# element36-io/hyperfridge-r0

Hardware: AMD Instinct MI355X
Metric: segments/sec (po2=20) proving camt53 guest, 1/2/4/8 MI355X (higher is better)
Workload: dtype u32

## Files before the change

hyperfridge-r0_amd/csrc/circuit.hip:

```cpp
#include <hip/hiprtc.h>

#include <memory>

#include "circuit.hpp"

namespace r0h {

static const char* compile_in_process(const std::string& src, std::vector<char>& code) {
  hiprtcProgram prog;
  hiprtcResult r = hiprtcCreateProgram(&prog, src.c_str(), "eval_check.hip", 0, nullptr, nullptr);
  R0H_REQUIRE(r == HIPRTC_SUCCESS, "hiprtcCreateProgram: %s", hiprtcGetErrorString(r));
  const char* opts[] = {"--offload-arch=gfx950", "-O3"};
  r = hiprtcCompileProgram(prog, 2, opts);
  if (r != HIPRTC_SUCCESS) {
    size_t n = 0;
    hiprtcGetProgramLogSize(prog, &n);
    std::string log(n, 0);
    if (n) hiprtcGetProgramLog(prog, &log[0]);
    hiprtcDestroyProgram(&prog);
    return make_error("hiprtcCompileProgram: %s\n%.2000s", hiprtcGetErrorString(r), log.c_str());
  }
  size_t n = 0;
  hiprtcGetCodeSize(prog, &n);
  code.resize(n);
// ... 80 lines not shown
  kernels_out->swap(kernels);
  return nullptr;
}

const char* r0h_circuit_load(r0h_ctx* ctx, const uint32_t* blob, size_t n_words, const char* code_object_path, r0h_circuit** out) {
  R0H_GUARD_BEGIN
  R0H_REQUIRE(ctx && blob && out, "r0h_circuit_load: NULL argument");
  std::unique_ptr<r0h_circuit, CircuitUnload> c(new r0h_circuit());
  c->ctx = ctx;
  R0H_TRY(parse_blob(c.get(), blob, n_words));
  make_plan(c.get());
  R0H_TRY(load_module("r0h_circuit_load", c.get(), code_object_path, emit_source, "eval_check", c->plan.terms.empty() ? 0 : 1, true, &c->module, &c->kernels));
  ctx_retain(ctx);
  *out = c.release();
  return nullptr;
  R0H_GUARD_END
}

const char* r0h_circuit_free(r0h_circuit* c) {
  if (!c) return nullptr;
  r0h_ctx* ctx = c->ctx;
  (void)hipSetDevice(ctx->device);
  (void)hipStreamSynchronize(ctx->stream);
  CircuitUnload()(c);
  ctx_release(ctx);
  return nullptr;
}

uint32_t r0h_circuit_group_size(const r0h_circuit* c, uint32_t group) { return c && group < 3 ? c->group_size[group] : 0; }
uint32_t r0h_circuit_n_global(const r0h_circuit* c) { return c ? c->n_global : 0; }
uint32_t r0h_circuit_n_mix(const r0h_circuit* c) { return c ? c->n_mix : 0; }
uint32_t r0h_circuit_n_taps(const r0h_circuit* c) { return c ? (uint32_t)c->taps.size() : 0; }
uint32_t r0h_circuit_n_terms(const r0h_circuit* c) { return c ? (uint32_t)c->plan.terms.size() : 0; }

static const char* check_module_load(const r0h_circuit* c, const char* caller, const char* code_object_path) {
  if (c->check_module) return nullptr;
  return load_module(caller, c, code_object_path, emit_check_source, "check_witness", c->plan.cut.size() - 1, false, &c->check_module, &c->check_kernels);
}

const char* r0h_circuit_load_check(r0h_circuit* c, const char* code_object_path) {
  R0H_GUARD_BEGIN
  R0H_REQUIRE(c, "r0h_circuit_load_check: NULL argument");
  std::lock_guard<std::mutex> lk(c->check_mu);
  R0H_REQUIRE(!c->check_module, "r0h_circuit_load_check: the circuit's checker is loaded already");
  return check_module_load(c, "r0h_circuit_load_check", code_object_path);
  R0H_GUARD_END
// ... 23 lines not shown
  const size_t table_at = kinds.size();
  for (uint32_t v : c->periodic) kinds.push_back(enc(v));
  R0H_TRY(ensure_scratch(ctx, kinds.size() * 4));
  R0H_TRY(stage_h2d(ctx, ctx->scratch, kinds.data(), kinds.size() * 4));
  const uint32_t* dk = (const uint32_t*)ctx->scratch;
  hipLaunchKernelGGL(witgen_fixed_kernel, dim3(n / threads, cols), dim3(threads), 0, ctx->stream, u32(buf), dk, po2, seed_mixed, dk + table_at, c->period);
  return launch_ok("r0h_witgen");
}
const char* witgen_code(r0h_ctx* ctx, const r0h_circuit* c, uint32_t po2, r0h_buf* code) {
  R0H_REQUIRE(ctx && c && code, "r0h_witgen: NULL argument");
  R0H_REQUIRE(c->has_column_program, "r0h_witgen: this circuit carries no synthetic column program (WITGEN/ACCUM sections); supply the witness");
  R0H_REQUIRE(po2 >= 4 && po2 <= R0H_MAX_PO2, "r0h_witgen: po2 %u outside [4, %u]", po2, R0H_MAX_PO2);
  const uint32_t nc = (uint32_t)c->code_cols.size();
  R0H_REQUIRE(((size_t)nc << po2) * 4 <= code->bytes, "r0h_witgen: buffers too small for 2^%u rows", po2);
  std::vector<uint32_t> kinds(2 * (size_t)nc);
  for (uint32_t k = 0; k < nc; k++) { kinds[2 * k] = c->code_cols[k].kind; kinds[2 * k + 1] = code_col_arg(c->code_cols[k], k); }
  return witgen_fixed(ctx, c, po2, kinds, splitmix64(CODE_SEED), code);
}
const char* code_commit_of(r0h_ctx* ctx, const r0h_circuit* c, uint32_t po2, r0h_code_commit** out) {
  DevBuf code;
  R0H_TRY(code.alloc(ctx, ((size_t)c->group_size[R0H_GROUP_CODE] << po2) * 4));
  R0H_TRY(witgen_code(ctx, c, po2, code.get()));
  return r0h_code_commit_new(ctx, code.get(), c->group_size[R0H_GROUP_CODE], po2, out);
}
}
extern "C" {

static const char* witgen_impl(r0h_ctx* ctx, const r0h_circuit* c, uint32_t po2, uint64_t seed, const uint32_t* global_in, r0h_buf* code,
                               r0h_buf* data, uint32_t* global_out) {
  R0H_GUARD_BEGIN
  R0H_REQUIRE(ctx && c && code && data, "r0h_witgen: NULL argument");
  R0H_REQUIRE(c->has_column_program, "r0h_witgen: this circuit carries no synthetic column program (WITGEN/ACCUM sections); supply the witness");
  R0H_REQUIRE(po2 >= 4 && po2 <= R0H_MAX_PO2, "r0h_witgen: po2 %u outside [4, %u]", po2, R0H_MAX_PO2);
  const uint32_t n = 1u << po2, threads = n < 256 ? n : 256, nc = (uint32_t)c->code_cols.size(), nd = (uint32_t)c->data_cols.size();
  R0H_REQUIRE(((size_t)nc << po2) * 4 <= code->bytes && ((size_t)nd << po2) * 4 <= data->bytes, "r0h_witgen: buffers too small for 2^%u rows", po2);
  R0H_TRY(witgen_code(ctx, c, po2, code));
  std::vector<uint32_t> kinds(2 * (size_t)nd);
  for (uint32_t k = 0; k < nd; k++) { kinds[2 * k] = c->data_cols[k].kind == 0 ? 3u : 99u; kinds[2 * k + 1] = (2u << 16) | k; }
  R0H_TRY(witgen_fixed(ctx, c, po2, kinds, splitmix64(seed), data));
  if (c->has_sponge) {
    R0H_TRY(sponge_plant(ctx, c, po2, nullptr, 0, data));
    if (!global_in) {
      uint32_t digest[8];
      p2_hash_elems_host(p2_default(), nullptr, 0, digest);
      for (uint32_t j = 0; j < 8; j++) R0H_TRY(stage_h2d(ctx, u32(data) + ((size_t)c->global_cols[c->sponge_global + j] << po2), digest + j, 4));
    }
// ... 180 lines not shown
```

hyperfridge-r0_amd/csrc/ctx.cpp:

```cpp
#include <stdarg.h>

#include <exception>
#include <stdexcept>

#include "../../include/r0hip_poseidon2_consts.h"
#include "internal.hpp"

namespace r0h {

const char* make_error(const char* fmt, ...) {
  char tmp[1024];
  va_list ap;
  va_start(ap, fmt);
  vsnprintf(tmp, sizeof tmp, fmt, ap);
  va_end(ap);
  char* out = (char*)malloc(strlen(tmp) + 1);
  if (!out) return "r0hip: out of memory while formatting an error";
  strcpy(out, tmp);
  return out;
}

void fill_p2(P2Consts& k, const uint32_t* rc, const uint32_t* diag) {
  int fr = 0, pr = 0;
  for (int r = 0; r < P2_ROUNDS; r++) {
// ... 185 lines not shown
  if (offset_bytes > b->bytes || bytes > b->bytes - offset_bytes) throw std::out_of_range("buf_view: window outside its buffer");
  r0h_buf v;
  v.ctx = b->ctx; v.ptr = (char*)b->ptr + offset_bytes; v.bytes = bytes; v.owned = false;
  return v;
}

const char* launch_ok(const char* what) {
  hipError_t e = hipGetLastError();
  R0H_REQUIRE(e == hipSuccess, "%s: launch failed: %s", what, hipGetErrorString(e));
  return nullptr;
}

void ctx_retain(r0h_ctx* ctx) { ctx->refs++; }
const char* ctx_helper(r0h_ctx* ctx, size_t k, r0h_ctx** out) {
  while (ctx->helpers.size() <= k) {
    r0h_ctx* h = nullptr;
    R0H_TRY(r0h_ctx_create(ctx->device, &h));
    ctx->helpers.push_back(h);
  }
  r0h_ctx* h = ctx->helpers[k];
  h->check_witness = ctx->check_witness;
  h->check_balance = ctx->check_balance;
  h->check_session = ctx->check_session;
  if (memcmp(&h->p2_host, &ctx->p2_host, sizeof(P2Consts)) != 0) {
    h->p2_host = ctx->p2_host;
    R0H_TRY_HIP(hipSetDevice(h->device));
    R0H_TRY_HIP(hipStreamSynchronize(h->stream));
    R0H_TRY_HIP(hipMemcpy(h->p2, &h->p2_host, sizeof(P2Consts), hipMemcpyHostToDevice));
  }
  *out = h;
  return nullptr;
}
void ctx_release(r0h_ctx* ctx) {
  if (--ctx->refs > 0) return;
  session_rows_free(ctx);
  for (r0h_ctx* h : ctx->helpers) r0h_ctx_destroy(h);
  ctx->helpers.clear();
  (void)hipSetDevice(ctx->device);
  (void)hipStreamSynchronize(ctx->stream);
  for (int d = 0; d < 2; d++) { (void)hipFree(ctx->tw_lo[d]); (void)hipFree(ctx->tw_hi[d]); (void)hipFree(ctx->tw12[d]); }
  for (int d = 0; d < 2; d++) { (void)hipFree(ctx->twb_lo[d]); (void)hipFree(ctx->twb_hi[d]); }
  (void)hipFree(ctx->pow3_lo); (void)hipFree(ctx->pow3_hi); (void)hipFree(ctx->pow3_top); (void)hipFree(ctx->p2); (void)hipFree(ctx->scratch);
  (void)hipHostFree(ctx->pinned);
  for (auto& kv : ctx->pool) (void)hipFree(kv.second);
  for (hipEvent_t e : ctx->prof.events) (void)hipEventDestroy(e);
  for (auto& kv : ctx->ktimers)
// ... 37 lines not shown
    R0H_TRY(upload_pow_table(&ctx->twb_hi[d], fpow(w26, TWB_SIZE), TWB_SIZE));
    R0H_TRY(upload_pow_table(&ctx->tw_lo[d], w22, TW_SIZE));
    R0H_TRY(upload_pow_table(&ctx->tw_hi[d], fpow(w22, TW_SIZE), TW_SIZE));
    R0H_TRY(upload_pow_table(&ctx->tw12[d], d == 0 ? rou_fwd(TWL_BITS) : rou_rev(TWL_BITS), 1u << (TWL_BITS - 1)));
  }
  R0H_TRY(upload_pow_table(&ctx->pow3_lo, enc(3), TW_SIZE));
  R0H_TRY(upload_pow_table(&ctx->pow3_hi, fpow(enc(3), TW_SIZE), TW_SIZE));
  R0H_TRY(upload_pow_table(&ctx->pow3_top, fpow(enc(3), (uint64_t)1 << TW_TOP), 1u << (MAX_DOMAIN_PO2 - TW_TOP)));
  R0H_TRY_HIP(hipMalloc((void**)&ctx->p2, sizeof(P2Consts)));
  ctx->p2_host = p2_default();
  R0H_TRY_HIP(hipMemcpy(ctx->p2, &ctx->p2_host, sizeof(P2Consts), hipMemcpyHostToDevice));
  ctx->pinned_bytes = 8u << 20;
  R0H_TRY_HIP(hipHostMalloc(&ctx->pinned, ctx->pinned_bytes, hipHostMallocDefault));
  R0H_TRY(ensure_scratch(ctx, 4u << 20));
  *out = ctx;
  return nullptr;
  R0H_GUARD_END
}

const char* r0h_ctx_destroy(r0h_ctx* ctx) {
  if (!ctx) return nullptr;
  (void)hipSetDevice(ctx->device);
  (void)hipStreamSynchronize(ctx->stream);
  ctx_release(ctx);
  return nullptr;
}

const char* r0h_sync(r0h_ctx* ctx) {
  R0H_REQUIRE(ctx, "r0h_sync: ctx is NULL");
  R0H_TRY_HIP(hipStreamSynchronize(ctx->stream));
  return nullptr;
}

const char* r0h_poseidon2_set_consts(r0h_ctx* ctx, const uint32_t* rc, const uint32_t* diag_m1) {
  R0H_REQUIRE(ctx && rc && diag_m1, "r0h_poseidon2_set_consts: NULL argument");
  for (int i = 0; i < P2_CELLS * P2_ROUNDS; i++) R0H_REQUIRE(rc[i] < P, "round constant %d not canonical", i);
  for (int i = 0; i < P2_CELLS; i++) R0H_REQUIRE(diag_m1[i] < P, "diagonal word %d not canonical", i);
  fill_p2(ctx->p2_host, rc, diag_m1);
  R0H_TRY_HIP(hipStreamSynchronize(ctx->stream));
  R0H_TRY_HIP(hipMemcpy(ctx->p2, &ctx->p2_host, sizeof(P2Consts), hipMemcpyHostToDevice));
  return nullptr;
}

const char* r0h_buf_alloc(r0h_ctx* ctx, size_t bytes, r0h_buf** out) {
  R0H_GUARD_BEGIN
  R0H_REQUIRE(ctx && out, "r0h_buf_alloc: NULL argument");
// ... 134 lines not shown
```

hyperfridge-r0_amd/csrc/hash_suite.cpp:

```cpp
#include "internal.hpp"
#include "receipt_types.hpp"

namespace r0h {
namespace {

inline uint32_t bswap(uint32_t x) { return __builtin_bswap32(x); }

void sha_compress(uint32_t st[8], const uint32_t* in) {
  uint32_t w[16];
  for (int i = 0; i < 16; i++) w[i] = bswap(in[i]);
  sha256_compress(st, w);
}

struct P2Rng : SuiteRng {
  const P2Consts* k;
  uint32_t cells[P2_CELLS];
  uint32_t pool_used = 0;
  explicit P2Rng(const P2Consts* kk) : k(kk) { memset(cells, 0, sizeof cells); }
  void mix(const uint32_t digest[8]) override {
    if (pool_used != 0) { p2_mix_host(*k, cells); pool_used = 0; }
    for (int i = 0; i < 8; i++) cells[i] = add(cells[i], digest[i]);
    p2_mix_host(*k, cells);
  }
  uint32_t elem() override {
// ... 89 lines not shown
  return nullptr;
}
std::unique_ptr<HashSuite> make_suite(int fn, const P2Consts* k) {
  if (fn == HASH_SHA256) return std::unique_ptr<HashSuite>(new ShaSuite());
  return std::unique_ptr<HashSuite>(new P2Suite(k));
}
const char* require_poseidon2(const r0h_ctx* ctx, const char* caller) {
  R0H_REQUIRE(ctx && ctx->hashfn == HASH_POSEIDON2,
              "%s: the context's hash suite is %s; receipts, sessions, image proofs and recursion nodes are poseidon2 only "
              "(r0h_ctx_set_hashfn(ctx, \"poseidon2\"))", caller, ctx ? hashfn_name(ctx->hashfn) : "unset (NULL context)");
  return nullptr;
}

}

using namespace r0h;

extern "C" {

const char* r0h_ctx_set_hashfn(r0h_ctx* ctx, const char* name) {
  R0H_REQUIRE(ctx, "r0h_ctx_set_hashfn: NULL argument");
  int fn = 0;
  R0H_TRY(hashfn_parse("r0h_ctx_set_hashfn", name, &fn));
  ctx->hashfn = fn;
  return nullptr;
}
const char* r0h_ctx_hashfn(const r0h_ctx* ctx) { return ctx ? hashfn_name(ctx->hashfn) : "poseidon2"; }

const char* r0h_hash_pair_host(const char* hashfn, const uint32_t a[8], const uint32_t b[8], uint32_t out[8]) {
  R0H_GUARD_BEGIN
  R0H_REQUIRE(a && b && out, "r0h_hash_pair_host: NULL argument");
  int fn = 0;
  R0H_TRY(hashfn_parse("r0h_hash_pair_host", hashfn, &fn));
  if (fn == HASH_POSEIDON2)
    for (int i = 0; i < 8; i++) R0H_REQUIRE(a[i] < P && b[i] < P, "r0h_hash_pair_host: word %d is not a canonical field element", i);
  make_suite(fn, &p2_default())->hash_pair(a, b, out);
  return nullptr;
  R0H_GUARD_END
}

const char* r0h_hash_elems_host(const char* hashfn, const uint32_t* words, size_t n, uint32_t out[8]) {
  R0H_GUARD_BEGIN
  R0H_REQUIRE((words || n == 0) && out, "r0h_hash_elems_host: NULL argument");
  int fn = 0;
  R0H_TRY(hashfn_parse("r0h_hash_elems_host", hashfn, &fn));
  if (fn == HASH_POSEIDON2)
// ... 8 lines not shown
```

hyperfridge-r0_amd/csrc/internal.hpp:

```cpp
#pragma once
#include <hip/hip_runtime.h>
#include <stdint.h>
#include <stdio.h>
#include <stdlib.h>
#include <string.h>

#include <map>
#include <memory>
#include <string>
#include <vector>

#include "../../include/r0hip.h"
#include "fp.hpp"

namespace r0h {

const char* make_error(const char* fmt, ...);

#define R0H_TRY_HIP(expr)                                                                              \
  do {                                                                                                 \
    hipError_t e__ = (expr);                                                                           \
    if (e__ != hipSuccess) return r0h::make_error("%s:%d: %s: %s", __FILE__, __LINE__, #expr, hipGetErrorString(e__)); \
  } while (0)
#define R0H_TRY(expr)                \
  do {                               \
    const char* m__ = (expr);        \
    if (m__) return m__;             \
  } while (0)
#define R0H_REQUIRE(cond, ...)                        \
  do {                                                \
    if (!(cond)) return r0h::make_error(__VA_ARGS__); \
  } while (0)
// ... 53 lines not shown
  uint32_t* pow3_hi = nullptr;
  uint32_t* pow3_top = nullptr;
  r0h::P2Consts* p2 = nullptr;
  r0h::P2Consts p2_host;
  int hashfn = 0;
  void* scratch = nullptr;
  size_t scratch_bytes = 0;
  void* pinned = nullptr;
  size_t pinned_bytes = 0, pinned_off = 0;
  std::multimap<size_t, void*> pool;
  size_t pool_bytes = 0;
  r0h::Profile prof;
  r0h_session_stats session = {0, 0, 0, 0, 0, 0, 0};
  const r0h_circuit* image_circuit = nullptr;
  uint64_t session_resident_limit = 0;
  void* session_rows = nullptr;
  std::vector<r0h_ctx*> helpers;
  bool check_witness = false;
  bool check_balance = false;
  bool check_session = false;
  uint64_t balance_stats[3] = {0, 0, 0};
  bool ktime_on = false;
  std::map<std::string, r0h::KTimer> ktimers;
};

struct r0h_buf {
  r0h_ctx* ctx = nullptr;
  void* ptr = nullptr;
  size_t bytes = 0;
  r0h_buf* parent = nullptr;
  int refs = 1;
  bool owned = true;
  bool pooled = false;
};

namespace r0h {
inline uint32_t* u32(const r0h_buf* b) { return (uint32_t*)b->ptr; }
struct KScope {
  r0h_ctx* ctx;
  KTimer* t = nullptr;
  KScope(r0h_ctx* c, const char* name, double alg_bytes) : ctx(c) {
    (void)hipSetDevice(c->device);
    if (!c->ktime_on) return;
    t = &c->ktimers[name];
    if (t->ev.size() < t->used + 2) {
      hipEvent_t a, b;
// ... 14 lines not shown
const char* ensure_scratch(r0h_ctx* ctx, size_t bytes);
const char* stage_h2d(r0h_ctx* ctx, void* dst_device, const void* src_host, size_t bytes);
const char* buf_alloc_pooled(r0h_ctx* ctx, size_t bytes, r0h_buf** out);
struct BufFree { void operator()(r0h_buf* b) const { r0h_buf_free(b); } };
struct DevBuf : std::unique_ptr<r0h_buf, BufFree> {
  const char* alloc(r0h_ctx* ctx, size_t bytes) {
    r0h_buf* b = nullptr;
    R0H_TRY(buf_alloc_pooled(ctx, bytes, &b));
    reset(b);
    return nullptr;
  }
};
r0h_buf buf_view(const r0h_buf* b, size_t offset_bytes, size_t bytes);
const char* launch_ok(const char* what);
const char* interpolate_ntt(r0h_ctx* ctx, r0h_buf* io, const r0h_buf* src, uint32_t count, uint32_t po2, bool zk_shift);
const char* evaluate_any(r0h_ctx* ctx, const r0h_buf* coeffs, uint32_t po2, const uint32_t* which, const uint32_t* xs, uint32_t n_eval,
                         r0h_buf* out, bool bitrev_coeffs);
const char* bit_reverse_ext(r0h_ctx* ctx, r0h_buf* io, uint32_t count, uint32_t po2);
const char* ntt_init_device();
const char* poly_divide_batch(r0h_ctx* ctx, r0h_buf* polys, uint32_t n, const uint32_t* poly_idx, const uint32_t* points, uint32_t n_jobs, uint32_t* remainders_host);
const char* unpack_ext_columns(r0h_ctx* ctx, uint32_t* cols, const uint32_t* packed, uint32_t po2);
const char* witgen_code(r0h_ctx* ctx, const r0h_circuit* c, uint32_t po2, r0h_buf* code);
const char* code_commit_of(r0h_ctx* ctx, const r0h_circuit* c, uint32_t po2, r0h_code_commit** out);
void vm_take_trace(r0h_vm* vm, size_t i, std::vector<r0h_preflight_row>& rows, std::vector<r0h_preflight_bound>& bounds);
void vm_recycle_trace(r0h_vm* vm, std::vector<r0h_preflight_row>& rows, std::vector<r0h_preflight_bound>& bounds);
void vm_take_spares(r0h_vm* vm, std::vector<std::vector<r0h_preflight_row>>& rows, std::vector<std::vector<r0h_preflight_bound>>& bounds);
void session_rows_free(r0h_ctx* ctx);
const char* ctx_helper(r0h_ctx* ctx, size_t k, r0h_ctx** out);
void ctx_retain(r0h_ctx* ctx);
void ctx_release(r0h_ctx* ctx);
void p2_mix_host(const P2Consts& k, uint32_t* cells);
void fill_p2(P2Consts& k, const uint32_t* rc, const uint32_t* diag_m1);
const P2Consts& p2_default();
void p2_hash_elems_host(const P2Consts& k, const uint32_t* elems, size_t n, uint32_t digest[8]);
void p2_sponge_rows_host(const P2Consts& k, const uint32_t* words, size_t n_words, uint32_t* cols, size_t stride, size_t* rows_used);

enum HashFn { HASH_POSEIDON2 = 0, HASH_SHA256 = 1 };
const char* hashfn_name(int fn);
const char* hashfn_parse(const char* caller, const char* name, int* fn_out);
struct SuiteRng {
  virtual ~SuiteRng() {}
  virtual void mix(const uint32_t digest[8]) = 0;
  virtual uint32_t elem() = 0;
  virtual uint32_t bits(uint32_t n) = 0;
  Fp4 ext() { Fp4 r; for (int i = 0; i < 4; i++) r.e[i] = elem(); return r; }
};
// ... 16 lines not shown
```

hyperfridge-r0_amd/csrc/poseidon2.hip:

```cpp
#include "poseidon2_device.hpp"

namespace r0h {

__global__ __launch_bounds__(256) void hash_rows_kernel(uint32_t* __restrict__ digests, const uint32_t* __restrict__ matrix,
                                                         uint32_t rows, uint32_t cols, const P2Consts* __restrict__ k) {
  uint32_t row = blockIdx.x * 256 + threadIdx.x;
  if (row >= rows) return;
  uint32_t c[P2_CELLS];
#pragma unroll
  for (int i = 0; i < P2_CELLS; i++) c[i] = 0;
  const uint32_t* src = matrix + row;
  uint32_t full = cols / P2_RATE, rem = cols % P2_RATE;
  for (uint32_t blk = 0; blk < full; blk++) {
#pragma unroll
    for (int i = 0; i < P2_RATE; i++) c[i] = src[(size_t)(blk * P2_RATE + i) * rows];
    p2_mix(c, k);
  }
  if (rem != 0 || cols == 0) {
#pragma unroll
    for (int i = 0; i < P2_RATE; i++) c[i] = (uint32_t)i < rem ? src[(size_t)(full * P2_RATE + i) * rows] : 0u;
    p2_mix(c, k);
  }
  uint4* dst = (uint4*)(digests + (size_t)row * 8);
  dst[0] = make_uint4(c[0], c[1], c[2], c[3]);
  dst[1] = make_uint4(c[4], c[5], c[6], c[7]);
}

__global__ __launch_bounds__(256) void hash_fold_kernel(uint32_t* __restrict__ nodes, uint32_t output_size,
                                                         const P2Consts* __restrict__ k) {
  uint32_t t = blockIdx.x * 256 + threadIdx.x;
  if (t >= output_size) return;
  uint32_t i = output_size + t;
  const uint4* src = (const uint4*)(nodes + (size_t)2 * i * 8);
  uint32_t c[P2_CELLS];
#pragma unroll
  for (int q = 0; q < 4; q++) {
    uint4 v = src[q];
    c[4 * q] = v.x; c[4 * q + 1] = v.y; c[4 * q + 2] = v.z; c[4 * q + 3] = v.w;
  }
#pragma unroll
  for (int q = 16; q < P2_CELLS; q++) c[q] = 0;
  p2_mix(c, k);
  uint4* dst = (uint4*)(nodes + (size_t)i * 8);
  dst[0] = make_uint4(c[0], c[1], c[2], c[3]);
  dst[1] = make_uint4(c[4], c[5], c[6], c[7]);
}

__device__ __forceinline__ uint32_t half_shfl(uint32_t v, uint32_t src_in_half) {
  return __shfl(v, (int)((threadIdx.x & 32u) | src_in_half), 64);
}
__device__ __forceinline__ uint32_t m_ext_lanes(uint32_t x, uint32_t l) {
  const uint32_t q = l & ~3u;
  uint32_t a = half_shfl(x, q), b = half_shfl(x, q | 1), d = half_shfl(x, q | 2), e = half_shfl(x, q | 3);
  uint32_t t0 = add(a, b), t1 = add(d, e);
  uint32_t t2 = add(add(b, b), t1), t3 = add(add(e, e), t0);
  uint32_t t1x2 = add(t1, t1), t0x2 = add(t0, t0);
  uint32_t t4 = add(add(t1x2, t1x2), t3), t5 = add(add(t0x2, t0x2), t2);
  uint32_t t6 = add(t3, t5), t7 = add(t2, t4);
  const uint32_t j = l & 3u;
  uint32_t y = j == 0 ? t6 : (j == 1 ? t5 : (j == 2 ? t7 : t4));
  uint32_t t = add(y, half_shfl(y, l ^ 4u));
  uint32_t s = add(t, add(half_shfl(t, (l + 8u) % 24u), half_shfl(t, (l + 16u) % 24u)));
  return add(y, s);
}
__global__ __launch_bounds__(256) void hash_fold_lanes_kernel(uint32_t* __restrict__ nodes, uint32_t output_size,
// ... 79 lines not shown
```

hyperfridge-r0_amd/csrc/poseidon2_device.hpp:

```cpp
#pragma once
#include "internal.hpp"

namespace r0h {

__device__ __forceinline__ uint32_t sbox7(uint32_t x) {
  uint32_t x2 = mul_lazy(x, x);
  uint32_t x3 = mul_lazy(x2, x);
  uint32_t x4 = reduce1(mul_lazy(x2, x2));
  return reduce1(mul_lazy(x3, x4));
}

#define R0H_ASM_ADD(r, a, b, x) "v_add_u32 " r ", " a ", " b "\n\tv_subrev_co_u32 " x ", vcc, 0x78000001, " r "\n\tv_cndmask_b32 " r ", " x ", " r ", vcc\n\t"
#if defined(__HIP_DEVICE_COMPILE__) && !defined(R0H_MEXT_PLAIN)
template <bool FIRST>
__device__ __forceinline__ void m4_block(uint32_t& c0, uint32_t& c1, uint32_t& c2, uint32_t& c3, uint32_t& s0, uint32_t& s1, uint32_t& s2, uint32_t& s3) {
  uint32_t o0, o1, o2, o3, t0, t1, t2, t3, u, x;
  asm(R0H_ASM_ADD("%8", "%14", "%15", "%13")
      R0H_ASM_ADD("%9", "%16", "%17", "%13")
      R0H_ASM_ADD("%12", "%15", "%15", "%13")
      R0H_ASM_ADD("%10", "%12", "%9", "%13")
      R0H_ASM_ADD("%12", "%17", "%17", "%13")
      R0H_ASM_ADD("%11", "%12", "%8", "%13")
      R0H_ASM_ADD("%9", "%9", "%9", "%13")
      R0H_ASM_ADD("%9", "%9", "%9", "%13")
      R0H_ASM_ADD("%3", "%9", "%11", "%13")
      R0H_ASM_ADD("%8", "%8", "%8", "%13")
      R0H_ASM_ADD("%8", "%8", "%8", "%13")
      R0H_ASM_ADD("%1", "%8", "%10", "%13")
      R0H_ASM_ADD("%0", "%11", "%1", "%13")
      R0H_ASM_ADD("%2", "%10", "%3", "%13")
      R0H_ASM_ADD("%4", "%4", "%0", "%13") R0H_ASM_ADD("%5", "%5", "%1", "%13") R0H_ASM_ADD("%6", "%6", "%2", "%13") R0H_ASM_ADD("%7", "%7", "%3", "%13")
      : "=&v"(o0), "=&v"(o1), "=&v"(o2), "=&v"(o3), "+v"(s0), "+v"(s1), "+v"(s2), "+v"(s3), "=&v"(t0), "=&v"(t1), "=&v"(t2), "=&v"(t3), "=&v"(u), "=&v"(x)
      : "v"(c0), "v"(c1), "v"(c2), "v"(c3)
      : "vcc");
  c0 = o0; c1 = o1; c2 = o2; c3 = o3;
}
__device__ __forceinline__ void m_ext(uint32_t (&c)[P2_CELLS]) {
  uint32_t s0 = 0, s1 = 0, s2 = 0, s3 = 0, x;
#pragma unroll
  for (int k = 0; k < P2_CELLS; k += 4) m4_block<false>(c[k], c[k + 1], c[k + 2], c[k + 3], s0, s1, s2, s3);
  asm(R0H_ASM_ADD("%0", "%0", "%25", "%24") R0H_ASM_ADD("%1", "%1", "%26", "%24") R0H_ASM_ADD("%2", "%2", "%27", "%24") R0H_ASM_ADD("%3", "%3", "%28", "%24")
      R0H_ASM_ADD("%4", "%4", "%25", "%24") R0H_ASM_ADD("%5", "%5", "%26", "%24") R0H_ASM_ADD("%6", "%6", "%27", "%24") R0H_ASM_ADD("%7", "%7", "%28", "%24")
      R0H_ASM_ADD("%8", "%8", "%25", "%24") R0H_ASM_ADD("%9", "%9", "%26", "%24") R0H_ASM_ADD("%10", "%10", "%27", "%24") R0H_ASM_ADD("%11", "%11", "%28", "%24")
      R0H_ASM_ADD("%12", "%12", "%25", "%24") R0H_ASM_ADD("%13", "%13", "%26", "%24") R0H_ASM_ADD("%14", "%14", "%27", "%24") R0H_ASM_ADD("%15", "%15", "%28", "%24")
      R0H_ASM_ADD("%16", "%16", "%25", "%24") R0H_ASM_ADD("%17", "%17", "%26", "%24") R0H_ASM_ADD("%18", "%18", "%27", "%24") R0H_ASM_ADD("%19", "%19", "%28", "%24")
      R0H_ASM_ADD("%20", "%20", "%25", "%24") R0H_ASM_ADD("%21", "%21", "%26", "%24") R0H_ASM_ADD("%22", "%22", "%27", "%24") R0H_ASM_ADD("%23", "%23", "%28", "%24")
      : "+v"(c[0]), "+v"(c[1]), "+v"(c[2]), "+v"(c[3]), "+v"(c[4]), "+v"(c[5]), "+v"(c[6]), "+v"(c[7]), "+v"(c[8]), "+v"(c[9]), "+v"(c[10]), "+v"(c[11]),
        "+v"(c[12]), "+v"(c[13]), "+v"(c[14]), "+v"(c[15]), "+v"(c[16]), "+v"(c[17]), "+v"(c[18]), "+v"(c[19]), "+v"(c[20]), "+v"(c[21]), "+v"(c[22]), "+v"(c[23]),
        "=&v"(x)
      : "v"(s0), "v"(s1), "v"(s2), "v"(s3)
      : "vcc");
}
#else
__device__ __forceinline__ void m_ext(uint32_t (&c)[P2_CELLS]) {
  uint32_t s0, s1, s2, s3;
#pragma unroll
  for (int k = 0; k < P2_CELLS; k += 4) {
    uint32_t a = c[k], b = c[k + 1], d = c[k + 2], e = c[k + 3];
    uint32_t t0 = add(a, b), t1 = add(d, e);
    uint32_t t2 = add(add(b, b), t1), t3 = add(add(e, e), t0);
    uint32_t t1x2 = add(t1, t1), t0x2 = add(t0, t0);
    uint32_t t4 = add(add(t1x2, t1x2), t3), t5 = add(add(t0x2, t0x2), t2);
    c[k] = add(t3, t5); c[k + 1] = t5; c[k + 2] = add(t2, t4); c[k + 3] = t4;
    if (k == 0) { s0 = c[0]; s1 = c[1]; s2 = c[2]; s3 = c[3]; }
    else { s0 = add(s0, c[k]); s1 = add(s1, c[k + 1]); s2 = add(s2, c[k + 2]); s3 = add(s3, c[k + 3]); }
  }
#pragma unroll
  for (int k = 0; k < P2_CELLS; k += 4) {
    c[k] = add(c[k], s0); c[k + 1] = add(c[k + 1], s1); c[k + 2] = add(c[k + 2], s2); c[k + 3] = add(c[k + 3], s3);
  }
}
#endif

__device__ __forceinline__ uint32_t sum_lanes_1_to_23(const uint32_t (&c)[P2_CELLS]) {
  uint32_t s1[12];
#pragma unroll
  for (int i = 0; i < 11; i++) s1[i] = add(c[2 * i + 2], c[2 * i + 3]);
  s1[11] = c[1];
  uint32_t s2[6];
#pragma unroll
  for (int i = 0; i < 6; i++) s2[i] = add(s1[2 * i], s1[2 * i + 1]);
  return add(add(add(s2[0], s2[1]), add(s2[2], s2[3])), add(s2[4], s2[5]));
}

__device__ __forceinline__ void p2_full_round(uint32_t (&c)[P2_CELLS], const uint32_t* __restrict__ rc) {
#pragma unroll
  for (int i = 0; i < P2_CELLS; i++) c[i] = sbox7(add(c[i], rc[i]));
  m_ext(c);
}

__device__ __forceinline__ void dot_fix(uint64_t& acc) {
  acc = ((uint64_t)reduce1((uint32_t)(acc >> 32)) << 32) | (uint32_t)acc;
  asm("" : "+v"(acc));
}
__device__ __forceinline__ void dot_mac(uint64_t& acc, uint32_t a, uint32_t b, int idx) {
  if (idx == 0) { acc = (uint64_t)a * b; return; }
  if (idx >= 4 && (idx & 1) == 0) dot_fix(acc);
  acc += (uint64_t)a * b;
}
__device__ __forceinline__ uint32_t dot_finish(uint64_t acc) {
  dot_fix(acc);
  return reduce64(acc);
}

__device__ __forceinline__ void p2_partial_rounds(uint32_t (&c)[P2_CELLS], const P2Consts* __restrict__ k) {
  uint32_t zero;
  asm volatile("s_mov_b32 %0, 0" : "=s"(zero));
  uint32_t sums[P2_PARTIAL];
  uint32_t s0 = c[0];
  uint32_t sigma = sum_lanes_1_to_23(c);
  const uint32_t* __restrict__ row = k->part_sigma + zero;
#pragma unroll
  for (int r = 0; r < P2_PARTIAL; r++) {
    if (r > 0) {
      uint64_t acc;
#pragma unroll
      for (int i = 0; i < P2_CELLS - 1; i++) dot_mac(acc, c[i + 1], row[i], i);
#pragma unroll
      for (int j = 0; j < r; j++) dot_mac(acc, sums[j], row[P2_CELLS - 1 + j], P2_CELLS - 1 + j);
      sigma = dot_finish(acc);
      row += P2_CELLS - 1 + r;
    }
    const uint32_t y = sbox7(add(s0, k->rc_partial[r]));
    sums[r] = add(y, sigma);
    s0 = add(sums[r], mul_const(y, k->diag_canon[0], k->diag_shoup[0]));
  }
  c[0] = s0;
#pragma unroll
  for (int i = 1; i < P2_CELLS; i++) {
    const uint32_t* __restrict__ f = k->part_final + zero + (i - 1) * (P2_PARTIAL + 1);
    uint64_t acc;
    dot_mac(acc, c[i], f[0], 0);
#pragma unroll
    for (int q = 0; q < P2_PARTIAL; q++) dot_mac(acc, sums[q], f[1 + q], 1 + q);
    c[i] = dot_finish(acc);
  }
}

__device__ __forceinline__ void p2_mix(uint32_t (&c)[P2_CELLS], const P2Consts* __restrict__ k) {
  m_ext(c);
#pragma unroll 1
  for (int r = 0; r < P2_HALF_FULL; r++) p2_full_round(c, k->rc_full[r]);
  p2_partial_rounds(c, k);
#pragma unroll 1
  for (int r = P2_HALF_FULL; r < 2 * P2_HALF_FULL; r++) p2_full_round(c, k->rc_full[r]);
}

}
```

hyperfridge-r0_amd/csrc/session.cpp:

```cpp
#include <stdlib.h>
#include <string.h>

#include <algorithm>
#include <atomic>
#include <chrono>
#include <condition_variable>
#include <deque>
#include <map>
#include <memory>
#include <mutex>
#include <thread>
#include <utility>
#include <vector>

#include "circuit.hpp"
#include "receipt_types.hpp"

using namespace r0h;

namespace {
using Clock = std::chrono::steady_clock;
double seconds(Clock::time_point a, Clock::time_point b) { return std::chrono::duration<double>(b - a).count(); }

struct CodeCommits {
  std::map<uint32_t, r0h_code_commit*> by_po2;
  ~CodeCommits() { for (auto& kv : by_po2) r0h_code_commit_free(kv.second); }
  const char* get(r0h_ctx* ctx, const r0h_circuit* c, uint32_t po2, r0h_code_commit** out) {
    auto it = by_po2.find(po2);
    if (it == by_po2.end()) {
      r0h_code_commit* cc = nullptr;
      R0H_TRY(code_commit_of(ctx, c, po2, &cc));
      it = by_po2.emplace(po2, cc).first;
    }
    *out = it->second;
    return nullptr;
  }
};

struct Produced {
  size_t index = 0;
  r0h_vm_segment info;
  r0h_receipt_claim claim;
  std::vector<r0h_preflight_row> rows;
  std::vector<r0h_preflight_bound> bounds;
};

uint32_t trace_size(uint64_t rows) {
  uint32_t po2 = 9;
  while (((uint64_t)1 << po2) < rows) po2++;
  return po2;
}

struct RowPool {
  std::mutex mu;
  std::vector<std::vector<r0h_preflight_row>> rows;
  std::vector<std::vector<r0h_preflight_bound>> bounds;
  std::map<const void*, size_t> pinned;
  ~RowPool() { settle(0); }
  void unpin(const void* p) {
    auto it = pinned.find(p);
// ... 213 lines not shown
  for (size_t k = 1; k < lanes.size(); k++) workers.emplace_back(lane, lanes[k]);
  lane(lanes[0]);
  for (std::thread& t : workers) t.join();
  return first;
}
}

namespace r0h {
void session_rows_free(r0h_ctx* ctx) {
  delete (RowPool*)ctx->session_rows;
  ctx->session_rows = nullptr;
}
}


constexpr uint32_t RECORD_WORDS = (R0H_TRACE_GLOBALS - R0H_TRACE_LATE_GLOBALS) + 8;
static_assert(RECORD_WORDS == R0H_SESSION_RECORD_WORDS, "R0H_SESSION_RECORD_WORDS out of step");

struct ProofAbort { void operator()(r0h_proof* p) const { r0h_proof_abort(p); } };

struct Pending {
  size_t index = 0;
  r0h_ctx* lctx = nullptr;
  DevBuf data;
  std::unique_ptr<r0h_proof, ProofAbort> proof;
  r0h_code_commit* cc = nullptr;
  uint32_t po2 = 0;
  std::vector<uint32_t> global;
  uint32_t root[8] = {0};
  r0h_receipt_claim claim;
  std::vector<uint32_t> seal;
  bool done = false;
};

struct r0h_session {
  r0h_ctx* ctx = nullptr;
  const r0h_circuit* c = nullptr;
  bool trace_mode = false;
  uint32_t part = 0, parts = 1;
  size_t n_segments = 0;
  std::mutex commit_mu, result_mu;
  std::vector<Pending> pending;
  CodeCommits commits;
  std::vector<uint8_t> journal;
  std::vector<uint8_t> elf;
  bool check_session = false;
  uint8_t image_id[32] = {0};
  uint64_t cycles = 0;
  r0h_session_stats stats = {0, 0, 0, 0, 0, 0, 0};
  uint64_t resident_limit = 0, resident_evaluations = 0;
  Clock::time_point t_begin;
  std::vector<r0h_ctx*> lane_ctx;
  ~r0h_session() {
    pending.clear();
    if (ctx) ctx_release(ctx);
  }
};

namespace {
const char* commit_segment(r0h_session* ses, RowBuffers& rows, const Produced& seg, DevBuf& data, std::vector<uint32_t>& global, Pending& pend) {
  const r0h_circuit* c = ses->c;
  const Clock::time_point t0 = Clock::now();
  rows.pin(seg.rows.data(), seg.rows.capacity() * sizeof(r0h_preflight_row));
  const r0h_trace_segment ts = {seg.info.index + 1, seg.info.closing, seg.info.pre.pc, 0};
  R0H_TRY(r0h_trace_witgen(pend.lctx, seg.rows.data(), seg.rows.size(), seg.bounds.data(), seg.bounds.size(), pend.po2, &ts, data.get(), global.data()));
  R0H_TRY(r0h_logup_multiplicities(pend.lctx, c, pend.po2, data.get(), global.data()));
// ... 44 lines not shown
  return nullptr;
}

const char* take_segments(r0h_session* ses, Feed& feed, RowBuffers& rows, r0h_ctx* lctx) {
  const r0h_circuit* c = ses->c;
  std::vector<uint32_t> seal, global(c->n_global);
  for (;;) {
    Feed::Segment seg;
    R0H_TRY(feed.next(seg));
    if (!seg) return nullptr;
    const uint64_t rows_needed = ses->trace_mode ? seg->rows.size() + seg->bounds.size() : seg->info.user_cycles + seg->info.paging_cycles;
    DevBuf data;
    Pending pend;
    pend.index = seg->index;
    pend.lctx = lctx;
    pend.claim = seg->claim;
    pend.po2 = trace_size(rows_needed);
    if (ses->trace_mode && pend.po2 < R0H_TRACE_MIN_PO2) pend.po2 = R0H_TRACE_MIN_PO2;
    uint8_t cd[32];
    claim_digest(seg->claim, cd);
    std::fill(global.begin(), global.end(), 0u);
    claim_globals(cd, global.data());
    R0H_TRY(data.alloc(lctx, ((size_t)c->group_size[R0H_GROUP_DATA] << pend.po2) * 4));
    {
      std::lock_guard<std::mutex> lk(ses->commit_mu);
      R0H_TRY(ses->commits.get(lctx, c, pend.po2, &pend.cc));
    }
    R0H_TRY(ses->trace_mode ? commit_segment(ses, rows, *seg, data, global, pend) : prove_synthetic_segment(ses, *seg, data, global, seal, pend));
  }
}

uint32_t lane_count() {
  uint32_t n = 2;
  if (const char* v = getenv("R0H_SESSION_LANES")) n = (uint32_t)strtoul(v, nullptr, 10);
  return n < 1 ? 1 : n > 4 ? 4 : n;
}
}

extern "C" {

const char* r0h_last_session_stats(r0h_ctx* ctx, r0h_session_stats* out) {
  R0H_REQUIRE(ctx && out, "r0h_last_session_stats: NULL argument");
  *out = ctx->session;
  return nullptr;
}

const char* r0h_session_free(r0h_session* s) {
  delete s;
  return nullptr;
}
// ... 215 lines not shown
```

Before: 41.17.

## Cache code commitments on the context and trim Poseidon2 first/last rounds

Moves the per-session code-commit cache into the circuit's owning context, keyed by circuit, po2 and hash function, so later sessions reuse code commitments instead of rebuilding them. Separately specialises the Poseidon2 external matrix: the first block skips adding to zero sums, zero-capacity absorbs skip the capacity blocks, and the final round of digest-only permutations writes just the first eight cells. It also tightens dot_fix to a single conditional subtract. This adds shared mutable state guarded by a mutex and cache invalidation when the hash function or round constants change.

```diff
diff --git a/hyperfridge-r0_amd/csrc/circuit.hip b/hyperfridge-r0_amd/csrc/circuit.hip
--- a/hyperfridge-r0_amd/csrc/circuit.hip
+++ b/hyperfridge-r0_amd/csrc/circuit.hip
@@ -126,6 +126,7 @@
   r0h_ctx* ctx = c->ctx;
   (void)hipSetDevice(ctx->device);
   (void)hipStreamSynchronize(ctx->stream);
+  ctx_code_commits_drop(ctx, c);
   CircuitUnload()(c);
   ctx_release(ctx);
   return nullptr;
@@ -195,6 +196,31 @@
   R0H_TRY(code.alloc(ctx, ((size_t)c->group_size[R0H_GROUP_CODE] << po2) * 4));
   R0H_TRY(witgen_code(ctx, c, po2, code.get()));
   return r0h_code_commit_new(ctx, code.get(), c->group_size[R0H_GROUP_CODE], po2, out);
+}
+const char* ctx_code_commit(r0h_ctx* lane, const r0h_circuit* c, uint32_t po2, std::shared_ptr<r0h_code_commit>* out) {
+  r0h_ctx* owner = c->ctx;
+  std::lock_guard<std::mutex> lk(owner->code_commits_mu);
+  const auto key = std::make_tuple(c, po2, lane->hashfn);
+  auto it = owner->code_commits.find(key);
+  if (it != owner->code_commits.end() && memcmp(&it->second.table, &lane->p2_host, sizeof(P2Consts)) != 0) {
+    owner->code_commits.erase(it);
+    it = owner->code_commits.end();
+  }
+  if (it == owner->code_commits.end()) {
+    r0h_code_commit* cc = nullptr;
+    R0H_TRY(code_commit_of(lane, c, po2, &cc));
+    std::shared_ptr<r0h_code_commit> held(cc, [](r0h_code_commit* p) { r0h_code_commit_free(p); });
+    it = owner->code_commits.emplace(key, r0h_ctx::CodeCommitEntry{held, lane->p2_host}).first;
+  }
+  *out = it->second.cc;
+  return nullptr;
+}
+void ctx_code_commits_drop(r0h_ctx* ctx, const r0h_circuit* c) {
+  std::lock_guard<std::mutex> lk(ctx->code_commits_mu);
+  for (auto it = ctx->code_commits.begin(); it != ctx->code_commits.end();) {
+    if (c && std::get<0>(it->first) != c) { ++it; continue; }
+    it = ctx->code_commits.erase(it);
+  }
 }
 }
 extern "C" {
diff --git a/hyperfridge-r0_amd/csrc/ctx.cpp b/hyperfridge-r0_amd/csrc/ctx.cpp
--- a/hyperfridge-r0_amd/csrc/ctx.cpp
+++ b/hyperfridge-r0_amd/csrc/ctx.cpp
@@ -231,6 +231,7 @@
   h->check_witness = ctx->check_witness;
   h->check_balance = ctx->check_balance;
   h->check_session = ctx->check_session;
+  h->hashfn = ctx->hashfn;
   if (memcmp(&h->p2_host, &ctx->p2_host, sizeof(P2Consts)) != 0) {
     h->p2_host = ctx->p2_host;
     R0H_TRY_HIP(hipSetDevice(h->device));
@@ -314,6 +315,7 @@
   if (!ctx) return nullptr;
   (void)hipSetDevice(ctx->device);
   (void)hipStreamSynchronize(ctx->stream);
+  ctx_code_commits_drop(ctx, nullptr);
   ctx_release(ctx);
   return nullptr;
 }
diff --git a/hyperfridge-r0_amd/csrc/hash_suite.cpp b/hyperfridge-r0_amd/csrc/hash_suite.cpp
--- a/hyperfridge-r0_amd/csrc/hash_suite.cpp
+++ b/hyperfridge-r0_amd/csrc/hash_suite.cpp
@@ -135,6 +135,7 @@
   R0H_REQUIRE(ctx, "r0h_ctx_set_hashfn: NULL argument");
   int fn = 0;
   R0H_TRY(hashfn_parse("r0h_ctx_set_hashfn", name, &fn));
+  if (fn != ctx->hashfn) ctx_code_commits_drop(ctx, nullptr);
   ctx->hashfn = fn;
   return nullptr;
 }
diff --git a/hyperfridge-r0_amd/csrc/internal.hpp b/hyperfridge-r0_amd/csrc/internal.hpp
--- a/hyperfridge-r0_amd/csrc/internal.hpp
+++ b/hyperfridge-r0_amd/csrc/internal.hpp
@@ -7,7 +7,9 @@
 
 #include <map>
 #include <memory>
+#include <mutex>
 #include <string>
+#include <tuple>
 #include <vector>
 
 #include "../../include/r0hip.h"
@@ -107,6 +109,9 @@
   uint64_t balance_stats[3] = {0, 0, 0};
   bool ktime_on = false;
   std::map<std::string, r0h::KTimer> ktimers;
+  struct CodeCommitEntry { std::shared_ptr<r0h_code_commit> cc; r0h::P2Consts table; };
+  std::mutex code_commits_mu;
+  std::map<std::tuple<const r0h_circuit*, uint32_t, int>, CodeCommitEntry> code_commits;
 };
 
 struct r0h_buf {
@@ -167,6 +172,8 @@
 const char* unpack_ext_columns(r0h_ctx* ctx, uint32_t* cols, const uint32_t* packed, uint32_t po2);
 const char* witgen_code(r0h_ctx* ctx, const r0h_circuit* c, uint32_t po2, r0h_buf* code);
 const char* code_commit_of(r0h_ctx* ctx, const r0h_circuit* c, uint32_t po2, r0h_code_commit** out);
+const char* ctx_code_commit(r0h_ctx* lane, const r0h_circuit* c, uint32_t po2, std::shared_ptr<r0h_code_commit>* out);
+void ctx_code_commits_drop(r0h_ctx* ctx, const r0h_circuit* c);
 void vm_take_trace(r0h_vm* vm, size_t i, std::vector<r0h_preflight_row>& rows, std::vector<r0h_preflight_bound>& bounds);
 void vm_recycle_trace(r0h_vm* vm, std::vector<r0h_preflight_row>& rows, std::vector<r0h_preflight_bound>& bounds);
 void vm_take_spares(r0h_vm* vm, std::vector<std::vector<r0h_preflight_row>>& rows, std::vector<std::vector<r0h_preflight_bound>>& bounds);
diff --git a/hyperfridge-r0_amd/csrc/poseidon2.hip b/hyperfridge-r0_amd/csrc/poseidon2.hip
--- a/hyperfridge-r0_amd/csrc/poseidon2.hip
+++ b/hyperfridge-r0_amd/csrc/poseidon2.hip
@@ -10,16 +10,12 @@
 #pragma unroll
   for (int i = 0; i < P2_CELLS; i++) c[i] = 0;
   const uint32_t* src = matrix + row;
-  uint32_t full = cols / P2_RATE, rem = cols % P2_RATE;
-  for (uint32_t blk = 0; blk < full; blk++) {
+  const uint32_t blocks = cols ? (cols + P2_RATE - 1) / P2_RATE : 1u;
+  for (uint32_t blk = 0; blk < blocks; blk++) {
+    const uint32_t have = cols - blk * P2_RATE;
 #pragma unroll
-    for (int i = 0; i < P2_RATE; i++) c[i] = src[(size_t)(blk * P2_RATE + i) * rows];
-    p2_mix(c, k);
-  }
-  if (rem != 0 || cols == 0) {
-#pragma unroll
-    for (int i = 0; i < P2_RATE; i++) c[i] = (uint32_t)i < rem ? src[(size_t)(full * P2_RATE + i) * rows] : 0u;
-    p2_mix(c, k);
+    for (int i = 0; i < P2_RATE; i++) c[i] = (uint32_t)i < have ? src[(size_t)(blk * P2_RATE + i) * rows] : 0u;
+    p2_mix_ends(c, k, blk == 0, blk + 1 == blocks);
   }
   uint4* dst = (uint4*)(digests + (size_t)row * 8);
   dst[0] = make_uint4(c[0], c[1], c[2], c[3]);
@@ -40,7 +36,7 @@
   }
 #pragma unroll
   for (int q = 16; q < P2_CELLS; q++) c[q] = 0;
-  p2_mix(c, k);
+  p2_mix<P2_ZERO_CAP | P2_DIGEST_ONLY>(c, k);
   uint4* dst = (uint4*)(nodes + (size_t)i * 8);
   dst[0] = make_uint4(c[0], c[1], c[2], c[3]);
   dst[1] = make_uint4(c[4], c[5], c[6], c[7]);
diff --git a/hyperfridge-r0_amd/csrc/poseidon2_device.hpp b/hyperfridge-r0_amd/csrc/poseidon2_device.hpp
--- a/hyperfridge-r0_amd/csrc/poseidon2_device.hpp
+++ b/hyperfridge-r0_amd/csrc/poseidon2_device.hpp
@@ -12,33 +12,67 @@
 
 #define R0H_ASM_ADD(r, a, b, x) "v_add_u32 " r ", " a ", " b "\n\tv_subrev_co_u32 " x ", vcc, 0x78000001, " r "\n\tv_cndmask_b32 " r ", " x ", " r ", vcc\n\t"
 #if defined(__HIP_DEVICE_COMPILE__) && !defined(R0H_MEXT_PLAIN)
+#define R0H_ASM_M4(T0, T1, T2, T3, U, X, A, B, D, E, O0, O1, O2, O3) \
+  R0H_ASM_ADD(T0, A, B, X)     \
+  R0H_ASM_ADD(T1, D, E, X)     \
+  R0H_ASM_ADD(U, B, B, X)      \
+  R0H_ASM_ADD(T2, U, T1, X)    \
+  R0H_ASM_ADD(U, E, E, X)      \
+  R0H_ASM_ADD(T3, U, T0, X)    \
+  R0H_ASM_ADD(T1, T1, T1, X)   \
+  R0H_ASM_ADD(T1, T1, T1, X)   \
+  R0H_ASM_ADD(O3, T1, T3, X)   \
+  R0H_ASM_ADD(T0, T0, T0, X)   \
+  R0H_ASM_ADD(T0, T0, T0, X)   \
+  R0H_ASM_ADD(O1, T0, T2, X)   \
+  R0H_ASM_ADD(O0, T3, O1, X)   \
+  R0H_ASM_ADD(O2, T2, O3, X)
 template <bool FIRST>
 __device__ __forceinline__ void m4_block(uint32_t& c0, uint32_t& c1, uint32_t& c2, uint32_t& c3, uint32_t& s0, uint32_t& s1, uint32_t& s2, uint32_t& s3) {
   uint32_t o0, o1, o2, o3, t0, t1, t2, t3, u, x;
-  asm(R0H_ASM_ADD("%8", "%14", "%15", "%13")
-      R0H_ASM_ADD("%9", "%16", "%17", "%13")
-      R0H_ASM_ADD("%12", "%15", "%15", "%13")
-      R0H_ASM_ADD("%10", "%12", "%9", "%13")
-      R0H_ASM_ADD("%12", "%17", "%17", "%13")
-      R0H_ASM_ADD("%11", "%12", "%8", "%13")
-      R0H_ASM_ADD("%9", "%9", "%9", "%13")
-      R0H_ASM_ADD("%9", "%9", "%9", "%13")
-      R0H_ASM_ADD("%3", "%9", "%11", "%13")
-      R0H_ASM_ADD("%8", "%8", "%8", "%13")
-      R0H_ASM_ADD("%8", "%8", "%8", "%13")
-      R0H_ASM_ADD("%1", "%8", "%10", "%13")
-      R0H_ASM_ADD("%0", "%11", "%1", "%13")
-      R0H_ASM_ADD("%2", "%10", "%3", "%13")
-      R0H_ASM_ADD("%4", "%4", "%0", "%13") R0H_ASM_ADD("%5", "%5", "%1", "%13") R0H_ASM_ADD("%6", "%6", "%2", "%13") R0H_ASM_ADD("%7", "%7", "%3", "%13")
-      : "=&v"(o0), "=&v"(o1), "=&v"(o2), "=&v"(o3), "+v"(s0), "+v"(s1), "+v"(s2), "+v"(s3), "=&v"(t0), "=&v"(t1), "=&v"(t2), "=&v"(t3), "=&v"(u), "=&v"(x)
-      : "v"(c0), "v"(c1), "v"(c2), "v"(c3)
+  if (FIRST) {
+    asm(R0H_ASM_M4("%4", "%5", "%6", "%7", "%8", "%9", "%10", "%11", "%12", "%13", "%0", "%1", "%2", "%3")
+        : "=&v"(o0), "=&v"(o1), "=&v"(o2), "=&v"(o3), "=&v"(t0), "=&v"(t1), "=&v"(t2), "=&v"(t3), "=&v"(u), "=&v"(x)
+        : "v"(c0), "v"(c1), "v"(c2), "v"(c3)
+        : "vcc");
+    s0 = o0; s1 = o1; s2 = o2; s3 = o3;
+  } else {
+    uint32_t n0, n1, n2, n3;
+    asm(R0H_ASM_M4("%8", "%9", "%10", "%11", "%12", "%13", "%14", "%15", "%16", "%17", "%0", "%1", "%2", "%3")
+        R0H_ASM_ADD("%4", "%18", "%0", "%13") R0H_ASM_ADD("%5", "%19", "%1", "%13") R0H_ASM_ADD("%6", "%20", "%2", "%13") R0H_ASM_ADD("%7", "%21", "%3", "%13")
+        : "=&v"(o0), "=&v"(o1), "=&v"(o2), "=&v"(o3), "=&v"(n0), "=&v"(n1), "=&v"(n2), "=&v"(n3), "=&v"(t0), "=&v"(t1), "=&v"(t2), "=&v"(t3), "=&v"(u), "=&v"(x)
+        : "v"(c0), "v"(c1), "v"(c2), "v"(c3), "v"(s0), "v"(s1), "v"(s2), "v"(s3)
+        : "vcc");
+    s0 = n0; s1 = n1; s2 = n2; s3 = n3;
+  }
+  c0 = o0; c1 = o1; c2 = o2; c3 = o3;
+}
+template <int N>
+__device__ __forceinline__ void add_sums(uint32_t (&c)[P2_CELLS], uint32_t s0, uint32_t s1, uint32_t s2, uint32_t s3);
+template <>
+__device__ __forceinline__ void add_sums<2>(uint32_t (&c)[P2_CELLS], uint32_t s0, uint32_t s1, uint32_t s2, uint32_t s3) {
+  uint32_t x;
+  asm(R0H_ASM_ADD("%0", "%0", "%9", "%8") R0H_ASM_ADD("%1", "%1", "%10", "%8") R0H_ASM_ADD("%2", "%2", "%11", "%8") R0H_ASM_ADD("%3", "%3", "%12", "%8")
+      R0H_ASM_ADD("%4", "%4", "%9", "%8") R0H_ASM_ADD("%5", "%5", "%10", "%8") R0H_ASM_ADD("%6", "%6", "%11", "%8") R0H_ASM_ADD("%7", "%7", "%12", "%8")
+      : "+v"(c[0]), "+v"(c[1]), "+v"(c[2]), "+v"(c[3]), "+v"(c[4]), "+v"(c[5]), "+v"(c[6]), "+v"(c[7]), "=&v"(x)
+      : "v"(s0), "v"(s1), "v"(s2), "v"(s3)
       : "vcc");
-  c0 = o0; c1 = o1; c2 = o2; c3 = o3;
-}
-__device__ __forceinline__ void m_ext(uint32_t (&c)[P2_CELLS]) {
-  uint32_t s0 = 0, s1 = 0, s2 = 0, s3 = 0, x;
-#pragma unroll
-  for (int k = 0; k < P2_CELLS; k += 4) m4_block<false>(c[k], c[k + 1], c[k + 2], c[k + 3], s0, s1, s2, s3);
+}
+template <>
+__device__ __forceinline__ void add_sums<4>(uint32_t (&c)[P2_CELLS], uint32_t s0, uint32_t s1, uint32_t s2, uint32_t s3) {
+  uint32_t x;
+  asm(R0H_ASM_ADD("%0", "%0", "%17", "%16") R0H_ASM_ADD("%1", "%1", "%18", "%16") R0H_ASM_ADD("%2", "%2", "%19", "%16") R0H_ASM_ADD("%3", "%3", "%20", "%16")
+      R0H_ASM_ADD("%4", "%4", "%17", "%16") R0H_ASM_ADD("%5", "%5", "%18", "%16") R0H_ASM_ADD("%6", "%6", "%19", "%16") R0H_ASM_ADD("%7", "%7", "%20", "%16")
+      R0H_ASM_ADD("%8", "%8", "%17", "%16") R0H_ASM_ADD("%9", "%9", "%18", "%16") R0H_ASM_ADD("%10", "%10", "%19", "%16") R0H_ASM_ADD("%11", "%11", "%20", "%16")
+      R0H_ASM_ADD("%12", "%12", "%17", "%16") R0H_ASM_ADD("%13", "%13", "%18", "%16") R0H_ASM_ADD("%14", "%14", "%19", "%16") R0H_ASM_ADD("%15", "%15", "%20", "%16")
+      : "+v"(c[0]), "+v"(c[1]), "+v"(c[2]), "+v"(c[3]), "+v"(c[4]), "+v"(c[5]), "+v"(c[6]), "+v"(c[7]), "+v"(c[8]), "+v"(c[9]), "+v"(c[10]), "+v"(c[11]),
+        "+v"(c[12]), "+v"(c[13]), "+v"(c[14]), "+v"(c[15]), "=&v"(x)
+      : "v"(s0), "v"(s1), "v"(s2), "v"(s3)
+      : "vcc");
+}
+template <>
+__device__ __forceinline__ void add_sums<6>(uint32_t (&c)[P2_CELLS], uint32_t s0, uint32_t s1, uint32_t s2, uint32_t s3) {
+  uint32_t x;
   asm(R0H_ASM_ADD("%0", "%0", "%25", "%24") R0H_ASM_ADD("%1", "%1", "%26", "%24") R0H_ASM_ADD("%2", "%2", "%27", "%24") R0H_ASM_ADD("%3", "%3", "%28", "%24")
       R0H_ASM_ADD("%4", "%4", "%25", "%24") R0H_ASM_ADD("%5", "%5", "%26", "%24") R0H_ASM_ADD("%6", "%6", "%27", "%24") R0H_ASM_ADD("%7", "%7", "%28", "%24")
       R0H_ASM_ADD("%8", "%8", "%25", "%24") R0H_ASM_ADD("%9", "%9", "%26", "%24") R0H_ASM_ADD("%10", "%10", "%27", "%24") R0H_ASM_ADD("%11", "%11", "%28", "%24")
@@ -51,7 +85,23 @@
       : "v"(s0), "v"(s1), "v"(s2), "v"(s3)
       : "vcc");
 }
+template <bool ZERO_CAP = false, bool DIGEST_ONLY = false>
+__device__ __forceinline__ void m_ext(uint32_t (&c)[P2_CELLS]) {
+  uint32_t s0, s1, s2, s3;
+  m4_block<true>(c[0], c[1], c[2], c[3], s0, s1, s2, s3);
+#pragma unroll
+  for (int k = 4; k < (ZERO_CAP ? P2_RATE : P2_CELLS); k += 4) m4_block<false>(c[k], c[k + 1], c[k + 2], c[k + 3], s0, s1, s2, s3);
+  if (DIGEST_ONLY) {
+    add_sums<2>(c, s0, s1, s2, s3);
+  } else if (ZERO_CAP) {
+    add_sums<4>(c, s0, s1, s2, s3);
+    c[16] = c[20] = s0; c[17] = c[21] = s1; c[18] = c[22] = s2; c[19] = c[23] = s3;
+  } else {
+    add_sums<6>(c, s0, s1, s2, s3);
+  }
+}
 #else
+template <bool ZERO_CAP = false, bool DIGEST_ONLY = false>
 __device__ __forceinline__ void m_ext(uint32_t (&c)[P2_CELLS]) {
   uint32_t s0, s1, s2, s3;
 #pragma unroll
@@ -83,14 +133,22 @@
   return add(add(add(s2[0], s2[1]), add(s2[2], s2[3])), add(s2[4], s2[5]));
 }
 
-__device__ __forceinline__ void p2_full_round(uint32_t (&c)[P2_CELLS], const uint32_t* __restrict__ rc) {
+__device__ __forceinline__ void p2_full_round(uint32_t (&c)[P2_CELLS], const uint32_t* __restrict__ rc, bool digest_only = false) {
 #pragma unroll
   for (int i = 0; i < P2_CELLS; i++) c[i] = sbox7(add(c[i], rc[i]));
-  m_ext(c);
+  if (digest_only) m_ext<false, true>(c);
+  else m_ext(c);
 }
 
 __device__ __forceinline__ void dot_fix(uint64_t& acc) {
-  acc = ((uint64_t)reduce1((uint32_t)(acc >> 32)) << 32) | (uint32_t)acc;
+  uint32_t hi = (uint32_t)(acc >> 32);
+#if defined(__HIP_DEVICE_COMPILE__)
+  uint32_t x;
+  asm("v_subrev_co_u32 %1, vcc, 0x78000001, %0\n\tv_cndmask_b32 %0, %1, %0, vcc" : "+v"(hi), "=&v"(x) : : "vcc");
+#else
+  hi = reduce1(hi);
+#endif
+  acc = ((uint64_t)hi << 32) | (uint32_t)acc;
   asm("" : "+v"(acc));
 }
 __device__ __forceinline__ void dot_mac(uint64_t& acc, uint32_t a, uint32_t b, int idx) {
@@ -137,13 +195,21 @@
   }
 }
 
-__device__ __forceinline__ void p2_mix(uint32_t (&c)[P2_CELLS], const P2Consts* __restrict__ k) {
-  m_ext(c);
+__device__ __forceinline__ void p2_mix_ends(uint32_t (&c)[P2_CELLS], const P2Consts* __restrict__ k, bool zero_cap, bool digest_only) {
+  if (zero_cap) m_ext<true, false>(c);
+  else m_ext(c);
 #pragma unroll 1
   for (int r = 0; r < P2_HALF_FULL; r++) p2_full_round(c, k->rc_full[r]);
   p2_partial_rounds(c, k);
 #pragma unroll 1
-  for (int r = P2_HALF_FULL; r < 2 * P2_HALF_FULL; r++) p2_full_round(c, k->rc_full[r]);
-}
-
-}
+  for (int r = P2_HALF_FULL; r < 2 * P2_HALF_FULL; r++) {
+    p2_full_round(c, k->rc_full[r], digest_only && r == 2 * P2_HALF_FULL - 1);
+  }
+}
+constexpr int P2_ZERO_CAP = 1, P2_DIGEST_ONLY = 2;
+template <int ENDS = 0>
+__device__ __forceinline__ void p2_mix(uint32_t (&c)[P2_CELLS], const P2Consts* __restrict__ k) {
+  p2_mix_ends(c, k, (ENDS & P2_ZERO_CAP) != 0, (ENDS & P2_DIGEST_ONLY) != 0);
+}
+
+}
diff --git a/hyperfridge-r0_amd/csrc/session.cpp b/hyperfridge-r0_amd/csrc/session.cpp
--- a/hyperfridge-r0_amd/csrc/session.cpp
+++ b/hyperfridge-r0_amd/csrc/session.cpp
@@ -21,21 +21,6 @@
 namespace {
 using Clock = std::chrono::steady_clock;
 double seconds(Clock::time_point a, Clock::time_point b) { return std::chrono::duration<double>(b - a).count(); }
-
-struct CodeCommits {
-  std::map<uint32_t, r0h_code_commit*> by_po2;
-  ~CodeCommits() { for (auto& kv : by_po2) r0h_code_commit_free(kv.second); }
-  const char* get(r0h_ctx* ctx, const r0h_circuit* c, uint32_t po2, r0h_code_commit** out) {
-    auto it = by_po2.find(po2);
-    if (it == by_po2.end()) {
-      r0h_code_commit* cc = nullptr;
-      R0H_TRY(code_commit_of(ctx, c, po2, &cc));
-      it = by_po2.emplace(po2, cc).first;
-    }
-    *out = it->second;
-    return nullptr;
-  }
-};
 
 struct Produced {
   size_t index = 0;
@@ -295,6 +280,7 @@
 struct Pending {
   size_t index = 0;
   r0h_ctx* lctx = nullptr;
+  std::shared_ptr<r0h_code_commit> cc_held;
   DevBuf data;
   std::unique_ptr<r0h_proof, ProofAbort> proof;
   r0h_code_commit* cc = nullptr;
@@ -312,9 +298,8 @@
   bool trace_mode = false;
   uint32_t part = 0, parts = 1;
   size_t n_segments = 0;
-  std::mutex commit_mu, result_mu;
+  std::mutex result_mu;
   std::vector<Pending> pending;
-  CodeCommits commits;
   std::vector<uint8_t> journal;
   std::vector<uint8_t> elf;
   bool check_session = false;
@@ -405,10 +390,8 @@
     std::fill(global.begin(), global.end(), 0u);
     claim_globals(cd, global.data());
     R0H_TRY(data.alloc(lctx, ((size_t)c->group_size[R0H_GROUP_DATA] << pend.po2) * 4));
-    {
-      std::lock_guard<std::mutex> lk(ses->commit_mu);
-      R0H_TRY(ses->commits.get(lctx, c, pend.po2, &pend.cc));
-    }
+    R0H_TRY(ctx_code_commit(lctx, c, pend.po2, &pend.cc_held));
+    pend.cc = pend.cc_held.get();
     R0H_TRY(ses->trace_mode ? commit_segment(ses, rows, *seg, data, global, pend) : prove_synthetic_segment(ses, *seg, data, global, seal, pend));
   }
 }
```

After: 42.37 (median of 6 runs). 2.9% higher.
